# apache/arrow

Hardware: AMD Instinct MI355X
Metric: filter_take_mrows_per_s (higher is better)
Workload: dtype int64; 1 GPU; Filter+Take int64[1000000000] + validity (10% null), boolean mask 10% true, FilterOptions::DROP; take indices = the mask's row numbers (monotonic; indices_nonzero: uint64 through CallFunction, GetTakeIndices: uint32 in the mirror), no boundscheck; inputs = splitmix64 streams of SURVEY.md 8(d) (seeds 1,2,3); rows=1000000000, selected_rows=99992053, parallelism=single-gpu

## Files before the change

### arrow_amd/_lib.py

```python
from __future__ import annotations

import ctypes as C
import os

_HERE = os.path.dirname(os.path.abspath(__file__))
LIB_PATH = os.path.join(_HERE, "libarrow_amd.so")

ARX_OK = 0
ARX_OUT_OF_MEMORY = -1
ARX_INVALID = -4
ARX_CAPACITY_ERROR = -6
ARX_INDEX_ERROR = -7
ARX_NOT_IMPLEMENTED = -10
ARX_DEVICE_ERROR = -100

ABI_VERSION = 5

FILTER_DROP, FILTER_EMIT_NULL = 0, 1
JOIN_COLUMN, JOIN_LITERAL, JOIN_NULL = 0, 1, 2
JOIN_NULL_HANDLING = {"emit_null": 0, "skip": 1, "replace": 2}
JOIN_MAX_OPERANDS = 32
CASE_WHEN_MAX_CONDS = 16
ELEMENT_WISE_MIN, ELEMENT_WISE_MAX = 0, 1
ELEMENT_WISE_MAX_OPERANDS = 32
# ... 84 lines not shown
        ("kind", C.c_int32),
        ("reserved", C.c_int32),
        ("column", ArxBinarySpan),
        ("literal", C.c_void_p),
        ("literal_length", C.c_int64),
    ]


_p, _i64, _int, _u64, _u32, _sz = C.c_void_p, C.c_int64, C.c_int, C.c_uint64, C.c_uint32, C.c_size_t
_span = C.POINTER(ArxSpan)
_bspan = C.POINTER(ArxBinarySpan)

SIGNATURES = {
    "arx_last_error": (C.c_char_p, []),
    "arx_abi_version": (_int, []),
    "arx_device_count": (_int, []),
    "arx_set_option": (_int, [C.c_char_p, _i64]),
    "arx_get_option": (_int, [C.c_char_p, C.POINTER(_i64)]),
    "arx_get_counter": (_i64, [C.c_char_p]),
    "arx_filter_workspace_bytes": (_sz, [_i64]),
    "arx_filter_count": (_int, [_span, _int, _p, _sz, C.POINTER(_i64), _p]),
    "arx_filter_count_async": (_int, [_span, _int, _p, _sz, _p]),
    "arx_filter_count_nulls": (_int, [_span, _span, _int, _p, _sz, C.POINTER(_i64), C.POINTER(_i64), _p]),
    "arx_filter_exec": (_int, [_span, _int, _span, _int, _p, _i64, _p, _p, _p]),
    "arx_mask_to_indices": (_int, [_span, _int, _p, _i64, _int, _p, _p, _p]),
    "arx_filter_compact_form": (_int, [_int, _int, _int, _int, _i64, _i64]),
    "arx_take_workspace_bytes": (_sz, []),
    "arx_check_index_bounds": (_int, [_span, _int, _u64, _p, _sz, _p]),
    "arx_take": (_int, [_span, _int, _span, _int, _p, _p, _p, _p]),
    "arx_take_rows": (_int, [_span, _i64, _span, _int, _p, _p, _p, _p]),
    "arx_take_bits": (_int, [_span, _span, _int, _p, _p, _p, _p]),
    "arx_binary_take_workspace_bytes": (_sz, [_i64]),
    "arx_binary_take_offsets": (_int, [_bspan, _span, _int, _p, _sz, _p, _p, _p, C.POINTER(_i64), _p]),
    "arx_binary_take_data": (_int, [_bspan, _i64, _p, _sz, _p, _i64, _p, _p]),
    "arx_large_binary_take_workspace_bytes": (_sz, [_i64]),
    "arx_large_binary_take_offsets": (_int, [_bspan, _span, _int, _p, _sz, _p, _p, _p, C.POINTER(_i64), _p]),
    "arx_large_binary_take_data": (_int, [_bspan, _i64, _p, _sz, _p, _i64, _p, _p]),
    "arx_list_take_data": (_int, [_bspan, _int, _i64, _p, _sz, _p, _i64, _p, _p]),
    "arx_large_list_take_data": (_int, [_bspan, _int, _i64, _p, _sz, _p, _i64, _p, _p]),
    "arx_plain_byte_array_offsets": (_int, [_p, _sz, _i64, C.c_int32, _p]),
    "arx_rle_scan_runs": (_int, [_p, _sz, _int, _i64, _u32, _u64, _p, _i64, C.POINTER(_i64), C.POINTER(_i64)]),
    "arx_rle_decode_u32": (_int, [_p, _sz, _p, _i64, _int, _i64, _p, _p]),
    "arx_rle_decode_equals_bitmap": (_int, [_p, _sz, _p, _i64, _int, _i64, _u32, _p, _p]),
    "arx_expand_by_mask": (_int, [_p, _int, _span, _p, _p, _p]),
    "arx_rle_levels_to_bitmap": (_int, [_p, _p, _i64, _p, _p, _p, _p]),
    "arx_rle_scan_runs_equals": (_int, [_p, _sz, _int, _i64, _u32, _u32, _u64, _p, _i64, C.POINTER(_i64), C.POINTER(_i64)]),
# ... 210 lines not shown
```

### arrow_amd/csrc/plugin/common.inc

```

std::atomic<int64_t> g_gpu_calls{0};
std::atomic<int64_t> g_stock_calls{0};
std::atomic<int64_t> g_min_rows{1 << 16};
std::atomic<int64_t> g_min_rows_streaming{INT64_MAX};
std::atomic<int64_t> g_filter_morsel_rows{[] {
  const char* env = std::getenv("ARROW_AMD_FILTER_MORSEL_ROWS");
  return env != nullptr ? static_cast<int64_t>(std::strtoll(env, nullptr, 10)) : int64_t(1) << 20;
}()};

std::atomic<bool> g_parquet_pinned_staging{true};
std::atomic<bool> g_parquet_device_levels{true};
std::atomic<int> g_parquet_read_threads{4};
std::atomic<int64_t> g_parquet_read_part_bytes{int64_t(1) << 23};
std::atomic<bool> g_parquet_device_snappy{[] {
  const char* env = std::getenv("ARROW_AMD_PARQUET_DEVICE_SNAPPY");
  return env == nullptr || std::strtoll(env, nullptr, 10) != 0;
}()};
std::atomic<int64_t> g_parquet_device_snappy_pages{0};
std::atomic<bool> g_parquet_device_gzip{true};
std::atomic<int64_t> g_parquet_device_gzip_pages{0};
std::atomic<int64_t> g_parquet_copied_pages{0};

std::atomic<int64_t> g_aggregate_flush_rows{[] {
  const char* env = std::getenv("ARROW_AMD_AGGREGATE_FLUSH_ROWS");
// ... 70 lines not shown
    case ARX_CAPACITY_ERROR: return Status::CapacityError(msg);
    case ARX_INDEX_ERROR: return Status::IndexError(msg);
    case ARX_NOT_IMPLEMENTED: return Status::NotImplemented(msg);
    case ARX_OUT_OF_MEMORY: return Status::OutOfMemory(msg);
    default: return Status::UnknownError(msg);
  }
}

#define HIP_RETURN_NOT_OK(call)                                                        \
  do {                                                                                 \
    hipError_t e__ = (call);                                                           \
    if (e__ != hipSuccess)                                                             \
      return Status::IOError("HIP: ", hipGetErrorString(e__), " in " #call);           \
  } while (0)

thread_local hipStream_t t_stream = nullptr;

class DeviceScratch {
 public:
  ~DeviceScratch() {
    for (auto& s : slots_) {
      if (s.ptr) (void)hipFree(s.ptr);
    }
  }
  hipStream_t PeekStream() const { return stream_; }
  Status Stream(hipStream_t* out) {
    if (!stream_) {
      HIP_RETURN_NOT_OK(hipStreamCreateWithFlags(&stream_, hipStreamNonBlocking));
      t_stream = stream_;
    }
    *out = stream_;
    return Status::OK();
  }
  Status Get(int slot, size_t bytes, void** out) {
    if (slots_.size() <= static_cast<size_t>(slot)) slots_.resize(slot + 1);
    Slot& s = slots_[slot];
    bytes = (bytes + 255) & ~size_t(255);
    if (s.size < bytes) {
      if (s.ptr) HIP_RETURN_NOT_OK(hipFree(s.ptr));
      s.ptr = nullptr;
      s.size = 0;
      const size_t want = std::max<size_t>(bytes + bytes / 4, 1 << 20);
      HIP_RETURN_NOT_OK(hipMalloc(&s.ptr, want));
      s.size = want;
    }
    *out = s.ptr;
    return Status::OK();
  }

 private:
  struct Slot { void* ptr = nullptr; size_t size = 0; };
  std::vector<Slot> slots_;
  hipStream_t stream_ = nullptr;
};
thread_local DeviceScratch t_scratch;

class PinnedStaging {
 public:
  ~PinnedStaging() {
    if (ptr_) (void)hipHostFree(ptr_);
  }
  Status Reserve(size_t bytes, uint8_t** out) {
    if (size_ < bytes) {
      if (ptr_) HIP_RETURN_NOT_OK(hipHostFree(ptr_));
      ptr_ = nullptr;
      size_ = 0;
      const size_t want = std::max<size_t>(bytes + bytes / 4, size_t(1) << 20);
      HIP_RETURN_NOT_OK(hipHostMalloc(&ptr_, want, hipHostMallocDefault));
      size_ = want;
    }
    *out = static_cast<uint8_t*>(ptr_);
    return Status::OK();
  }
  void Trim(size_t keep_at_most) {
    if (size_ > keep_at_most && ptr_ != nullptr) {
      (void)hipHostFree(ptr_);
      ptr_ = nullptr;
      size_ = 0;
// ... 106 lines not shown
```

### arrow_amd/csrc/plugin/selection.inc

```
StockKernel g_stock_filter;

arrow::Result<std::unique_ptr<cp::KernelState>> FilterInit(cp::KernelContext* ctx,
                                                           const cp::KernelInitArgs& args) {
  auto state = std::make_unique<ShimState<cp::FilterOptions>>();
  if (g_stock_filter.init) {
    ARROW_ASSIGN_OR_RAISE(state->stock, g_stock_filter.init(ctx, args));
  }
  if (args.options != nullptr) {
    state->options = *static_cast<const cp::FilterOptions*>(args.options);
  }
  return state;
}

Status BooleanTakeOnDevice(const ArxSpan& dv, const ArxSpan& di, int tid, hipStream_t st, ArrayData* out_arr) {
  const int64_t m = di.length;
  const int64_t bytes = ((m + 63) / 64) * 8;
  const bool allocate_validity = dv.null_count != 0 || di.null_count != 0;
  out_arr->length = m;
  out_arr->buffers.resize(2);
  out_arr->buffers[0] = nullptr;
  ARROW_ASSIGN_OR_RAISE(out_arr->buffers[1], AllocDevice(bytes));
  void* d_valid = nullptr;
  void* d_counter = nullptr;
  if (allocate_validity) {
    ARROW_ASSIGN_OR_RAISE(out_arr->buffers[0], AllocDevice(bytes));
    d_valid = reinterpret_cast<void*>(out_arr->buffers[0]->mutable_address());
    ARROW_RETURN_NOT_OK(t_scratch.Get(kCounter, 64, &d_counter));
    HIP_RETURN_NOT_OK(hipMemsetAsync(d_counter, 0, 8, st));
  }
  ARROW_RETURN_NOT_OK(FromArx(arx_take_bits(&dv, &di, tid, reinterpret_cast<void*>(out_arr->buffers[1]->mutable_address()),
                                            d_valid, static_cast<int64_t*>(d_counter), st)));
  int64_t valid_count = m;
  if (allocate_validity) HIP_RETURN_NOT_OK(hipMemcpyAsync(&valid_count, d_counter, 8, hipMemcpyDeviceToHost, st));
  HIP_RETURN_NOT_OK(hipStreamSynchronize(st));
  out_arr->null_count = m - valid_count;
  return Status::OK();
}

bool ReeFilterOnRocm(const ArraySpan& filter) {
  return filter.type->id() == Type::RUN_END_ENCODED && filter.child_data.size() == 2 &&
         OnRocm(filter.child_data[0]) && OnRocm(filter.child_data[1]);
}
Status ExpandReeFilterOnDevice(const ArraySpan& filter, hipStream_t st, ArxSpan* dm) {
  const ArraySpan& run_ends = filter.child_data[0];
  const ArraySpan& run_values = filter.child_data[1];
  const int rw = FixedByteWidth(*run_ends.type);
  if (run_values.type->id() != Type::BOOL || (rw != 2 && rw != 4 && rw != 8)) {
    return Status::NotImplemented("arrow_amd: filter of type ", filter.type->ToString());
  }
  ArxSpan ends{}, vals{};
  ARROW_RETURN_NOT_OK(DeviceSpan(run_ends, &ends));
  ARROW_RETURN_NOT_OK(DeviceSpan(run_values, &vals));
  const int64_t n = filter.length;
  const size_t bytes = static_cast<size_t>((n + 63) / 64) * 8 + 64;
  void *d_bits = nullptr, *d_valid = nullptr;
  ARROW_RETURN_NOT_OK(t_scratch.Get(kArg2, bytes, &d_bits));
  const bool may_have_nulls = vals.validity != nullptr && vals.null_count != 0;
  if (may_have_nulls) ARROW_RETURN_NOT_OK(t_scratch.Get(kArg2Validity, bytes, &d_valid));
// ... 56 lines not shown
      ARROW_RETURN_NOT_OK(ExpandReeFilterOnDevice(filter, st, &dm));
    } else {
      ARROW_RETURN_NOT_OK(DeviceSpan(filter, &dm));
    }
    const size_t ws_bytes = arx_filter_workspace_bytes(filter.length);
    void* ws = nullptr;
    ARROW_RETURN_NOT_OK(t_scratch.Get(kWs, ws_bytes, &ws));
    ArrayData* out_arr = out->array_data().get();
    const bool allocate_validity = dv.null_count != 0 || dm.null_count != 0;
    if (filter.length > 0 && filter.length <= g_filter_morsel_rows.load()) {
      const int64_t n = filter.length;
      ARROW_RETURN_NOT_OK(FromArx(arx_filter_count_async(&dm, null_sel, ws, ws_bytes, st)));
      out_arr->buffers.resize(2);
      ARROW_ASSIGN_OR_RAISE(out_arr->buffers[1], AllocDevice(n * w));
      out_arr->buffers[0] = nullptr;
      void* d_valid = nullptr;
      if (allocate_validity) {
        ARROW_ASSIGN_OR_RAISE(out_arr->buffers[0], AllocDevice(((n + 63) / 64) * 8));
        d_valid = reinterpret_cast<void*>(out_arr->buffers[0]->mutable_address());
      }
      ARROW_RETURN_NOT_OK(FromArx(arx_filter_exec(&dv, w, &dm, null_sel, ws, n,
                                                  reinterpret_cast<void*>(out_arr->buffers[1]->mutable_address()),
                                                  d_valid, st)));
      int64_t selected = 0, set_bits = 0;
      HIP_RETURN_NOT_OK(hipMemcpyAsync(&selected, ws, 8, hipMemcpyDeviceToHost, st));
      if (allocate_validity) {
        void* cws = nullptr;
        ARROW_RETURN_NOT_OK(t_scratch.Get(kCounter, 64, &cws));
        ARROW_RETURN_NOT_OK(FromArx(arx_bitmap_popcount(d_valid, 0, n, cws, 64, &set_bits, st)));
      } else {
        HIP_RETURN_NOT_OK(hipStreamSynchronize(st));
      }
      out_arr->length = selected;
      out_arr->null_count = allocate_validity ? selected - set_bits : 0;
      static_cast<RocmBuffer*>(out_arr->buffers[1].get())->Shrink(selected * w);
      if (allocate_validity) static_cast<RocmBuffer*>(out_arr->buffers[0].get())->Shrink(((selected + 63) / 64) * 8);
      CountGpu(kFnFilter);
      return Status::OK();
    }
    int64_t out_len = 0, out_nulls = 0;
    if (allocate_validity) {
      ARROW_RETURN_NOT_OK(FromArx(arx_filter_count_nulls(&dv, &dm, null_sel, ws, ws_bytes, &out_len, &out_nulls, st)));
    } else {
      ARROW_RETURN_NOT_OK(FromArx(arx_filter_count(&dm, null_sel, ws, ws_bytes, &out_len, st)));
    }
    out_arr->length = out_len;
    out_arr->buffers.resize(2);
    ARROW_ASSIGN_OR_RAISE(out_arr->buffers[1], AllocDevice(out_len * w));
    out_arr->buffers[0] = nullptr;
    void* d_valid = nullptr;
    if (allocate_validity) {
      ARROW_ASSIGN_OR_RAISE(out_arr->buffers[0], AllocDevice(((out_len + 63) / 64) * 8));
      d_valid = reinterpret_cast<void*>(out_arr->buffers[0]->mutable_address());
    }
    ARROW_RETURN_NOT_OK(FromArx(arx_filter_exec(&dv, w, &dm, null_sel, ws, out_len,
                                                reinterpret_cast<void*>(out_arr->buffers[1]->mutable_address()),
                                                d_valid, st)));
    out_arr->null_count = allocate_validity ? out_nulls : 0;
    HIP_RETURN_NOT_OK(hipStreamSynchronize(st));
    CountGpu(kFnFilter);
    return Status::OK();
  }
  if (w == 0 || filter.type->id() != Type::BOOL || values.length < g_min_rows.load() ||
      !IsHost(values) || !IsHost(filter)) {
    return RunStock(kFnFilter, g_stock_filter, state->stock.get(), ctx, batch, out);
  }
  hipStream_t st;
  ARROW_RETURN_NOT_OK(t_scratch.Stream(&st));
// ... 258 lines not shown
    }
    if (w == 0 || tid < 0) {
      return Status::NotImplemented("arrow_amd: take of ", values.type->ToString(), " by ",
                                    indices.type->ToString(), " on device-resident arrays");
    }
    hipStream_t st;
    ARROW_RETURN_NOT_OK(t_scratch.Stream(&st));
    ArxSpan dv{}, di{};
    ARROW_RETURN_NOT_OK(DeviceSpan(values, &dv));
    ARROW_RETURN_NOT_OK(DeviceSpan(indices, &di));
    if (state->options.boundscheck) ARROW_RETURN_NOT_OK(CheckBoundsOnDevice(di, tid, values.length, st));
    const int64_t m = indices.length;
    const bool allocate_validity = dv.null_count != 0 || di.null_count != 0;
    ArrayData* out_arr = out->array_data().get();
    out_arr->length = m;
    out_arr->buffers.resize(2);
    ARROW_ASSIGN_OR_RAISE(out_arr->buffers[1], AllocDevice(m * w));
    out_arr->buffers[0] = nullptr;
    void* d_valid = nullptr;
    void* d_counter = nullptr;
    if (allocate_validity) {
      ARROW_ASSIGN_OR_RAISE(out_arr->buffers[0], AllocDevice(((m + 63) / 64) * 8));
      d_valid = reinterpret_cast<void*>(out_arr->buffers[0]->mutable_address());
      ARROW_RETURN_NOT_OK(t_scratch.Get(kCounter, 64, &d_counter));
      HIP_RETURN_NOT_OK(hipMemsetAsync(d_counter, 0, 8, st));
    }
    ARROW_RETURN_NOT_OK(FromArx(arx_take(&dv, w, &di, tid,
                                         reinterpret_cast<void*>(out_arr->buffers[1]->mutable_address()), d_valid,
                                         static_cast<int64_t*>(d_counter), st)));
    int64_t valid_count = m;
    if (allocate_validity) {
      HIP_RETURN_NOT_OK(hipMemcpyAsync(&valid_count, d_counter, 8, hipMemcpyDeviceToHost, st));
    }
    HIP_RETURN_NOT_OK(hipStreamSynchronize(st));
    out_arr->null_count = m - valid_count;
    CountGpu(kFnTake);
    return Status::OK();
  }
  if (w == 0 || tid < 0 || indices.length < g_min_rows.load() || !IsHost(values) || !IsHost(indices)) {
    return RunStock(kFnTake, g_stock_take, state->stock.get(), ctx, batch, out);
  }
  hipStream_t st;
  ARROW_RETURN_NOT_OK(t_scratch.Stream(&st));
  ArxSpan dv{}, di{};
  ARROW_RETURN_NOT_OK(Upload(values, w, kValues, kValidity, st, &dv));
  ARROW_RETURN_NOT_OK(Upload(indices, kIdxWidth[tid], kArg2, kArg2Validity, st, &di));
  if (state->options.boundscheck) ARROW_RETURN_NOT_OK(CheckBoundsOnDevice(di, tid, values.length, st));
  const int64_t m = indices.length;
  const bool allocate_validity = values.MayHaveNulls() || indices.MayHaveNulls();
  ArrayData* out_arr = out->array_data().get();
  out_arr->length = m;
  out_arr->buffers.resize(2);
  ARROW_ASSIGN_OR_RAISE(out_arr->buffers[1], ctx->Allocate(m * w));
  void* d_out = nullptr;
  void* d_out_valid = nullptr;
  void* d_counter = nullptr;
  ARROW_RETURN_NOT_OK(t_scratch.Get(kOutData, static_cast<size_t>(m) * w + 16, &d_out));
  if (allocate_validity) {
// ... 24 lines not shown
```

### arrow_amd/csrc/plugin/vector_hash.inc

```
enum HashVectorKind { kHashUnique = 0, kHashValueCounts, kHashDictEncode };

struct DeviceHashState : public cp::KernelState {
  HashVectorKind kind = kHashUnique;
  std::unique_ptr<cp::KernelState> stock;
  bool used_stock = false, used_device = false;
  bool encode_nulls = false;
  std::shared_ptr<arrow::DataType> type;
  int width = 0;
  std::shared_ptr<Buffer> table_buf, counts_buf;
  void* table = nullptr;
  int64_t max_groups = 0, num_groups = 0, counts_cap = 0;
};

StockKernel g_stock_unique, g_stock_value_counts, g_stock_dict_encode;
cp::VectorKernel::FinalizeFunc g_stock_unique_finalize = nullptr, g_stock_value_counts_finalize = nullptr,
                               g_stock_dict_encode_finalize = nullptr;

template <HashVectorKind KIND>
const StockKernel& StockHashKernel() {
  return KIND == kHashUnique ? g_stock_unique : KIND == kHashValueCounts ? g_stock_value_counts : g_stock_dict_encode;
}

Status HashUniques(DeviceHashState* s, hipStream_t st, std::shared_ptr<Buffer>* values, std::shared_ptr<Buffer>* validity,
                   int64_t* null_count) {
// ... 293 lines not shown
  } else {
    const int num = NonZeroNumericTypeId(in.type->id());
    if (num < 0) return Status::NotImplemented("arrow_amd: indices_nonzero of device-resident ", in.type->ToString(), " arrays");
    static const int widths[10] = {1, 1, 2, 2, 4, 4, 8, 8, 4, 8};
    ARROW_ASSIGN_OR_RAISE(bits, AllocDevice(((n + 63) / 64) * 8 + 8));
    const uint64_t zero = 0;
    const uint8_t* base = static_cast<const uint8_t*>(dv.data) + dv.offset * widths[num];
    if (n > 0) {
      ARROW_RETURN_NOT_OK(FromArx(arx_compare_numeric(ARX_CMP_NOT_EQUAL, num, base, nullptr, nullptr, &zero, n,
                                                      reinterpret_cast<uint64_t*>(bits->mutable_address()), st)));
    }
    dm.data = reinterpret_cast<const void*>(bits->address());
    dm.offset = 0;
    if (dm.validity != nullptr && dv.offset != 0) {
      ARROW_ASSIGN_OR_RAISE(rebased, AllocDevice(((n + 63) / 64) * 8 + 8));
      ARROW_RETURN_NOT_OK(FromArx(arx_bitmap_copy(dv.validity, dv.offset, n, reinterpret_cast<void*>(rebased->mutable_address()), st)));
      dm.validity = reinterpret_cast<const void*>(rebased->address());
    }
  }
  const size_t ws_bytes = arx_filter_workspace_bytes(n);
  void* ws = nullptr;
  ARROW_RETURN_NOT_OK(t_scratch.Get(kWs, ws_bytes, &ws));
  int64_t cnt = 0;
  if (n > 0) ARROW_RETURN_NOT_OK(FromArx(arx_filter_count(&dm, ARX_FILTER_DROP, ws, ws_bytes, &cnt, st)));
  void* d_idx = nullptr;
  ARROW_RETURN_NOT_OK(t_scratch.Get(kArg2, static_cast<size_t>(cnt) * 4 + 64, &d_idx));
  ARROW_ASSIGN_OR_RAISE(auto out_values, AllocDevice(std::max<int64_t>(cnt, 1) * 8));
  bool direct = false;
  if (cnt > 0) {
    direct = arx_mask_to_indices(&dm, ARX_FILTER_DROP, ws, cnt, 8, reinterpret_cast<void*>(out_values->mutable_address()), nullptr, st) == ARX_OK;
  }
  if (cnt > 0 && !direct) {
    ARROW_RETURN_NOT_OK(FromArx(arx_mask_to_indices(&dm, ARX_FILTER_DROP, ws, cnt, 4, d_idx, nullptr, st)));
    ArxSpan di{nullptr, d_idx, 0, cnt, 0};
    void* flag = nullptr;
    ARROW_RETURN_NOT_OK(t_scratch.Get(kFlag, 64, &flag));
    ARROW_RETURN_NOT_OK(FromArx(arx_cast_numeric(&di, ARX_NUM_UINT32, ARX_NUM_UINT64, 1, 1, flag, 64,
                                                 reinterpret_cast<void*>(out_values->mutable_address()), st)));
  }
  HIP_RETURN_NOT_OK(hipStreamSynchronize(st));
  CountGpu(kFnFilter);
  out->value = ArrayData::Make(arrow::uint64(), cnt, {nullptr, std::move(out_values)}, 0);
  return Status::OK();
}

Status RegisterIndicesNonZero(cp::FunctionRegistry* reg) {
  ARROW_ASSIGN_OR_RAISE(auto fn, reg->GetFunction("indices_nonzero"));
  if (fn->kind() != cp::Function::VECTOR) return Status::Invalid("indices_nonzero is not a vector function");
  auto* vfn = static_cast<cp::VectorFunction*>(fn.get());
  for (const auto& ty : {arrow::boolean(), arrow::int8(), arrow::uint8(), arrow::int16(), arrow::uint16(), arrow::int32(),
                         arrow::uint32(), arrow::int64(), arrow::uint64(), arrow::float32(), arrow::float64()}) {
    ARROW_ASSIGN_OR_RAISE(const cp::Kernel* k0, vfn->DispatchExact({ty}));
    cp::VectorKernel copy = *static_cast<const cp::VectorKernel*>(k0);
    if (g_stock_nonzero.exec == nullptr) g_stock_nonzero.exec = copy.exec;
    if (g_stock_nonzero.exec != copy.exec) continue;
// ... 64 lines not shown
```

### arrow_amd/csrc/selection.hip

```cpp
#include "arx_common.h"

#include <string.h>

#include <algorithm>
#include <type_traits>

namespace arx {

struct FilterWsHeader {
  int64_t total;
  int64_t ntiles;
  int64_t ngroups;
  int64_t length;
  int64_t valid;
  int64_t pad[3];
};
static_assert(sizeof(FilterWsHeader) == 64, "header is one 64-byte line");

struct FilterWsView {
  FilterWsHeader* hdr;
  int64_t* group_excl;
  int64_t* group_total;
  uint32_t* tile_counts;
  int64_t* group_valid;
// ... 10 lines not shown
  uint8_t* p = static_cast<uint8_t*>(ws);
  v.hdr = reinterpret_cast<FilterWsHeader*>(p);
  v.group_excl = reinterpret_cast<int64_t*>(p + 64);
  v.group_total = v.group_excl + ng;
  v.tile_counts = reinterpret_cast<uint32_t*>(v.group_total + ng);
  v.group_valid = reinterpret_cast<int64_t*>(v.tile_counts + ng * kTilesPerGroup);
  return v;
}

__device__ __forceinline__ uint64_t emit_word(const Bits& mask, const Bits& mvalid, int64_t w,
                                              bool emit_null, bool invert,
                                              uint64_t* mask_valid_out) {
  uint64_t m = load_word(mask, w);
  const uint64_t mv = load_word(mvalid, w);
  *mask_valid_out = mv;
  if (emit_null || invert) {
    const uint64_t in_range = load_word(Bits{nullptr, 0, mask.length, 0}, w);
    if (invert) m = ~m & in_range;
    if (emit_null) return (m | ~mv) & in_range;
  }
  return m & mv;
}

template <bool VALID>
__global__ __launch_bounds__(kBlock) void count_kernel(Bits mask, Bits mvalid, Bits vvalid, int emit_null,
                                                       int invert, int64_t ntiles,
                                                       uint32_t* tile_counts,
                                                       int64_t* group_total, int64_t* group_valid) {
  __shared__ uint32_t wave_sums[kWavesPerBlock];
  __shared__ uint32_t wave_valid[kWavesPerBlock];
  const int lane = lane_id();
  const int wave = threadIdx.x >> 6;
  const int64_t group = blockIdx.x;
  const int64_t t0 = group * kTilesPerGroup + wave * 16;
  uint32_t mine = 0;
  uint32_t kv = 0;
#pragma unroll 4
  for (int i = 0; i < 16; ++i) {
    const int64_t t = t0 + i;
    uint32_t k = 0;
    if (t < ntiles) {
      uint64_t mv;
      const uint64_t e = emit_word(mask, mvalid, t * 64 + lane, emit_null != 0, invert != 0, &mv);
      k = __popcll(e);
      if constexpr (VALID) kv += __popcll(e & mv & load_word(vvalid, t * 64 + lane));
    }
    const uint32_t s = wave_reduce_sum_u32(k);
    if (lane == i) mine = s;
  }
  if (lane < 16) tile_counts[t0 + lane] = mine;
  const uint32_t wsum = wave_reduce_sum_u32(lane < 16 ? mine : 0u);
  if (lane == 0) wave_sums[wave] = wsum;
  if constexpr (VALID) {
    const uint32_t vsum = wave_reduce_sum_u32(kv);
    if (lane == 0) wave_valid[wave] = vsum;
  }
  __syncthreads();
  if (threadIdx.x == 0) {
    int64_t s = 0, v = 0;
    for (int i = 0; i < kWavesPerBlock; ++i) {
      s += wave_sums[i];
      if constexpr (VALID) v += wave_valid[i];
    }
    group_total[group] = s;
    if constexpr (VALID) group_valid[group] = v;
  }
}

__global__ __launch_bounds__(1024) void scan_kernel(const int64_t* group_total, int64_t ngroups,
                                                    int64_t* group_excl, FilterWsHeader* hdr,
                                                    const int64_t* group_valid = nullptr) {
  __shared__ int64_t wave_tot[16];
  __shared__ int64_t carry_s;
  __shared__ unsigned long long valid_s;
  const int tid = threadIdx.x;
  const int lane = tid & 63;
  const int wave = tid >> 6;
  if (tid == 0) carry_s = 0;
  if (tid == 0) valid_s = 0;
  __syncthreads();
  if (group_valid != nullptr) {
    int64_t mine = 0;
    for (int64_t i = tid; i < ngroups; i += 1024) mine += group_valid[i];
#pragma unroll
    for (int d = 32; d >= 1; d >>= 1) mine += __shfl_xor(mine, d, 64);
    if (lane == 0 && mine != 0) atomicAdd(&valid_s, static_cast<unsigned long long>(mine));
    __syncthreads();
  }
  for (int64_t base = 0; base < ngroups; base += 1024) {
    const int64_t i = base + tid;
    const int64_t v = i < ngroups ? group_total[i] : 0;
    int64_t x = v;
#pragma unroll
    for (int d = 1; d < 64; d <<= 1) {
      const int64_t n = __shfl_up(x, d, 64);
      if (lane >= d) x += n;
    }
    if (lane == 63) wave_tot[wave] = x;
    __syncthreads();
    int64_t wave_prefix = 0;
    for (int k = 0; k < wave; ++k) wave_prefix += wave_tot[k];
    const int64_t carry = carry_s;
    if (i < ngroups) group_excl[i] = carry + wave_prefix + x - v;
    __syncthreads();
    if (tid == 1023) carry_s = carry + wave_prefix + x;
    __syncthreads();
  }
  if (tid == 0) {
    hdr->total = carry_s;
    hdr->valid = static_cast<int64_t>(valid_s);
  }
}

struct CompactArgs {
  const uint8_t* values;
  Bits mask;
  Bits mvalid;
  Bits vvalid;
  int64_t length;
  int64_t ntiles;
  const uint32_t* tile_counts;
  const int64_t* group_excl;
  uint8_t* out_data;
  uint64_t* out_validity;
  int emit_null;
  int invert;
  int values_aligned16;
};

constexpr int kFlushBytes = 2048;

template <int RING>
struct __attribute__((aligned(16))) CompactLds {
// ... 377 lines not shown


constexpr int kSparseWindow = 1024;
constexpr int kSparseU = 2;

struct __attribute__((aligned(16))) SparseLds {
  uint16_t sel[kWavesPerBlock][kSparseWindow];
  uint64_t vs[kWavesPerBlock][64];
  uint64_t zw[kWavesPerBlock][64];
};

template <int W, bool EMIT, bool IOTA>
__global__ __launch_bounds__(kBlock) void compact_sparse_kernel(CompactArgs a) {
  using E = typename ElemT<W>::type;
  constexpr int U = kSparseU;
  __shared__ SparseLds lds;

  const int lane = lane_id();
  const int wave = __builtin_amdgcn_readfirstlane(threadIdx.x >> 6);
  const int64_t t = static_cast<int64_t>(blockIdx.x) * kWavesPerBlock + wave;
  if (t >= a.ntiles) return;

  const int64_t w = t * 64 + lane;
  uint64_t mv;
  const uint64_t Ew = emit_word(a.mask, a.mvalid, w, EMIT, a.invert != 0, &mv);
  const uint32_t k = __popcll(Ew);
  const uint32_t incl = wave_inclusive_scan_u32(k);
  const uint32_t p = incl - k;
  const int total = static_cast<int>(__shfl(incl, 63, 64));
  if (total == 0) return;

  const int64_t grp = t >> 6;
  const int tin = static_cast<int>(t & 63);
  const uint32_t cprev = lane < tin ? a.tile_counts[grp * kTilesPerGroup + lane] : 0u;
  const int64_t off = a.group_excl[grp] + wave_reduce_sum_u32(cprev);

  uint16_t* sel = lds.sel[wave];
  const bool want_validity = a.out_validity != nullptr;
  if (want_validity) lds.vs[wave][lane] = load_word(a.vvalid, w) & mv;
  if constexpr (EMIT) lds.zw[wave][lane] = Ew & ~mv;

  const E* __restrict__ values = IOTA ? nullptr : reinterpret_cast<const E*>(a.values) + t * kTileRows;
  E* __restrict__ out = reinterpret_cast<E*>(a.out_data);
  const int head = static_cast<int>(off & 63);
  const int nsteps = (head + total + 63) >> 6;
  const int64_t word0 = off >> 6;
  constexpr int kStepsPerWindow = kSparseWindow / 64;

  uint64_t m = Ew;
  uint32_t rk = p;
  for (int step0 = 0; step0 < nsteps; step0 += kStepsPerWindow) {
    const int win_lo = step0 * 64 - head;
    const int win_hi = win_lo + kSparseWindow;
    while (m != 0 && static_cast<int>(rk) < win_hi) {
      const int bpos = __ffsll(static_cast<unsigned long long>(m)) - 1;
      m &= m - 1;
      sel[static_cast<int>(rk) - win_lo] = static_cast<uint16_t>(lane * 64 + bpos);
      ++rk;
    }
    wave_lds_sync();
    const int step_end = (step0 + kStepsPerWindow) < nsteps ? (step0 + kStepsPerWindow) : nsteps;
    const int first_listed = win_lo < 0 ? 0 : win_lo;
// ... 438 lines not shown
  return ARX_OK;
}

static inline const void* effective_validity(const ArxSpan* s) {
  return (s->null_count != 0) ? s->validity : nullptr;
}

static int launch_count(const ArxSpan* mask, int null_selection, void* ws, size_t ws_bytes,
                        hipStream_t st, int invert = 0, const ArxSpan* values = nullptr) {
  const int rc = check_mask(mask, null_selection);
  if (rc != ARX_OK) return rc;
  const size_t need = arx_filter_workspace_bytes(mask->length);
  if (ws == nullptr || ws_bytes < need) {
    set_error("filter workspace too small: %zu < %zu", ws_bytes, need);
    return ARX_INVALID;
  }
  if ((reinterpret_cast<uint64_t>(ws) & 63) != 0) {
    set_error("filter workspace must be 64-byte aligned");
    return ARX_INVALID;
  }
  FilterWsView v = ws_view(ws, mask->length);
  const int64_t nt = num_tiles(mask->length);
  const int64_t ng = num_groups(mask->length);
  FilterWsHeader h{};
  h.total = 0;
  h.ntiles = nt;
  h.ngroups = ng;
  h.length = mask->length;
  ARX_HIP(hipMemcpyAsync(v.hdr, &h, sizeof(h), hipMemcpyHostToDevice, st));
  if (mask->length == 0) return ARX_OK;
  const Bits mb = make_bits(mask->data, mask->offset, mask->length);
  const Bits mvb = make_bits(effective_validity(mask), mask->offset, mask->length);
  if (values != nullptr) {
    const Bits vvb = make_bits(effective_validity(values), values->offset, mask->length);
    hipLaunchKernelGGL((count_kernel<true>), dim3(static_cast<unsigned>(ng)), dim3(kBlock), 0, st, mb, mvb, vvb,
                       null_selection, invert, nt, v.tile_counts, v.group_total, v.group_valid);
    ARX_CHECK_LAUNCH("count_kernel");
    hipLaunchKernelGGL(scan_kernel, dim3(1), dim3(1024), 0, st, v.group_total, ng, v.group_excl, v.hdr,
                       static_cast<const int64_t*>(v.group_valid));
  } else {
    hipLaunchKernelGGL((count_kernel<false>), dim3(static_cast<unsigned>(ng)), dim3(kBlock), 0, st, mb, mvb, mvb,
                       null_selection, invert, nt, v.tile_counts, v.group_total, static_cast<int64_t*>(nullptr));
    ARX_CHECK_LAUNCH("count_kernel");
    hipLaunchKernelGGL(scan_kernel, dim3(1), dim3(1024), 0, st, v.group_total, ng, v.group_excl, v.hdr,
                       static_cast<const int64_t*>(nullptr));
  }
  ARX_CHECK_LAUNCH("scan_kernel");
  return ARX_OK;
}

static Knob<int> g_filter_batch{4};
static Knob<int> g_filter_pipe{1};
static Knob<int> g_filter_sparse{-1};
static const KnobRow kSelectionKnobs[] = {
    {"filter_batch", g_filter_batch, knob_snap_down<1, 4>},
    {"filter_pipe", g_filter_pipe, knob_bool},
    {"filter_sparse", g_filter_sparse, knob_tri},
};
KnobTable selection_knobs() { return knob_table(kSelectionKnobs); }

template <int W, bool IOTA, bool EMIT, bool ALIGNED>
static void launch_compact_e(const CompactArgs& a, unsigned grid, hipStream_t st) {
  constexpr int kIters = kTileRows / (kWave * (16 / W));
  constexpr int kBig = kIters >= 8 ? 4 : 2;
  if (ALIGNED && g_filter_batch >= 4 && g_filter_pipe) {
    hipLaunchKernelGGL((compact_kernel<W, IOTA, EMIT, ALIGNED, kBig, true>), dim3(grid),
                       dim3(kBlock), 0, st, a);
  } else {
    hipLaunchKernelGGL((compact_kernel<W, IOTA, EMIT, ALIGNED, 1, false>), dim3(grid), dim3(kBlock),
// ... 140 lines not shown
  a.emit_null = 0;
  a.invert = invert ? 1 : 0;
  a.values_aligned16 = 1;
  return launch_compact(true, 4, a, st);
}

}

using namespace arx;

extern "C" {

size_t arx_filter_workspace_bytes(int64_t length) {
  if (length < 0) length = 0;
  const int64_t ng = num_groups(length);
  return static_cast<size_t>(64 + ng * 16 + ng * kTilesPerGroup * 4 + ng * 8 + 64);
}

int arx_filter_count_async(const ArxSpan* mask, int null_selection, void* ws, size_t ws_bytes,
                           void* stream) {
  return launch_count(mask, null_selection, ws, ws_bytes, as_stream(stream));
}

int arx_filter_count_nulls(const ArxSpan* values, const ArxSpan* mask, int null_selection, void* ws, size_t ws_bytes,
                           int64_t* out_length, int64_t* out_null_count, void* stream) {
  if (out_length == nullptr || out_null_count == nullptr || values == nullptr) {
    set_error("values / out_length / out_null_count is NULL");
    return ARX_INVALID;
  }
  if (mask != nullptr && values->length != mask->length) {
    set_error("filter values and mask differ in length (%lld vs %lld)", static_cast<long long>(values->length),
              static_cast<long long>(mask->length));
    return ARX_INVALID;
  }
  hipStream_t st = as_stream(stream);
  const int rc = launch_count(mask, null_selection, ws, ws_bytes, st, 0, values);
  if (rc != ARX_OK) return rc;
  int64_t hdr[5] = {0, 0, 0, 0, 0};
  ARX_HIP(hipMemcpyAsync(hdr, ws, sizeof(hdr), hipMemcpyDeviceToHost, st));
  ARX_HIP(hipStreamSynchronize(st));
  *out_length = hdr[0];
  *out_null_count = mask->length == 0 ? 0 : hdr[0] - hdr[4];
  return ARX_OK;
}

int arx_filter_count(const ArxSpan* mask, int null_selection, void* ws, size_t ws_bytes,
                     int64_t* out_length, void* stream) {
  if (out_length == nullptr) {
    set_error("out_length is NULL");
    return ARX_INVALID;
  }
  hipStream_t st = as_stream(stream);
  const int rc = launch_count(mask, null_selection, ws, ws_bytes, st);
  if (rc != ARX_OK) return rc;
  int64_t total = 0;
  ARX_HIP(hipMemcpyAsync(&total, ws, sizeof(int64_t), hipMemcpyDeviceToHost, st));
  ARX_HIP(hipStreamSynchronize(st));
  *out_length = total;
  return ARX_OK;
// ... 489 lines not shown
```

### include/arrow_amd.h

```cpp
#ifndef ARROW_AMD_H_
#define ARROW_AMD_H_

#include <stddef.h>
#include <stdint.h>

#ifdef __cplusplus
extern "C" {
#endif

#define ARX_ABI_VERSION 5

typedef enum ArxStatus {
  ARX_OK = 0,
  ARX_OUT_OF_MEMORY = -1,
  ARX_INVALID = -4,
  ARX_CAPACITY_ERROR = -6,
  ARX_INDEX_ERROR = -7,
  ARX_NOT_IMPLEMENTED = -10,
  ARX_DEVICE_ERROR = -100
} ArxStatus;

enum { ARX_FILTER_DROP = 0, ARX_FILTER_EMIT_NULL = 1 };
enum { ARX_SORT_ASCENDING = 0, ARX_SORT_DESCENDING = 1 };
enum { ARX_NULLS_AT_START = 0, ARX_NULLS_AT_END = 1 };
// ... 9 lines not shown
  int64_t offset;
  int64_t length;
  int64_t null_count;
} ArxSpan;

const char* arx_last_error(void);
int arx_abi_version(void);
int arx_device_count(void);
int arx_set_option(const char* name, int64_t value);
int arx_get_option(const char* name, int64_t* out_value);
int64_t arx_get_counter(const char* name);


size_t arx_filter_workspace_bytes(int64_t length);

int arx_filter_count(const ArxSpan* mask, int null_selection, void* ws, size_t ws_bytes,
                     int64_t* out_length, void* stream);

int arx_filter_count_nulls(const ArxSpan* values, const ArxSpan* mask, int null_selection, void* ws, size_t ws_bytes,
                           int64_t* out_length, int64_t* out_null_count, void* stream);

int arx_filter_count_async(const ArxSpan* mask, int null_selection, void* ws,
                           size_t ws_bytes, void* stream);

int arx_filter_exec(const ArxSpan* values, int byte_width, const ArxSpan* mask,
                    int null_selection, const void* ws, int64_t out_length, void* out_data,
                    void* out_validity, void* stream);

int arx_mask_to_indices(const ArxSpan* mask, int null_selection, const void* ws,
                        int64_t out_length, int index_width, void* out_indices,
                        void* out_validity, void* stream);

enum { ARX_COMPACT_GATHER = 0, ARX_COMPACT_SWEEP_PIPELINED = 1, ARX_COMPACT_SWEEP_PLAIN = 2, ARX_COMPACT_SWEEP_UNALIGNED = 3 };

int arx_filter_compact_form(int row_numbers, int byte_width, int values_aligned16, int invert,
                            int64_t length, int64_t out_length);

size_t arx_take_workspace_bytes(void);

int arx_check_index_bounds(const ArxSpan* indices, int index_type, uint64_t upper_limit,
                           void* ws, size_t ws_bytes, void* stream);

int arx_take(const ArxSpan* values, int byte_width, const ArxSpan* indices, int index_type,
             void* out_data, void* out_validity, int64_t* valid_count, void* stream);

int arx_take_rows(const ArxSpan* values, int64_t row_bytes, const ArxSpan* indices, int index_type, void* out_data,
// ... 653 lines not shown
```

Baseline: 306,400 Mrows/s.

## Batch count-kernel loads, fold header init into scan, pin readbacks, elide counter memsets

Several changes land together. Device-to-host readbacks now go through a pinned host buffer instead of pageable stack variables. The host-to-device header copy is replaced by having the scan kernel write the whole header. The count kernel now issues its mask and validity word loads in batches of four tiles, and the scan kernel processes four groups per thread and folds the valid-count reduction into the same pass. The exec kernel also issues its tile-count and group-offset loads earlier, and a reusable device counter is re-zeroed after use so the next call can skip a memset. These aim to cut host-device synchronisation and transfer overhead and to raise memory-level parallelism in the count pass, at the cost of more code and more registers per thread.

```diff
diff --git a/arrow_amd/_lib.py b/arrow_amd/_lib.py
--- a/arrow_amd/_lib.py
+++ b/arrow_amd/_lib.py
@@ -130,6 +130,7 @@
     "arx_filter_count": (_int, [_span, _int, _p, _sz, C.POINTER(_i64), _p]),
     "arx_filter_count_async": (_int, [_span, _int, _p, _sz, _p]),
     "arx_filter_count_nulls": (_int, [_span, _span, _int, _p, _sz, C.POINTER(_i64), C.POINTER(_i64), _p]),
+    "arx_filter_count_nulls_async": (_int, [_span, _span, _int, _p, _sz, _p]),
     "arx_filter_exec": (_int, [_span, _int, _span, _int, _p, _i64, _p, _p, _p]),
     "arx_mask_to_indices": (_int, [_span, _int, _p, _i64, _int, _p, _p, _p]),
     "arx_filter_compact_form": (_int, [_int, _int, _int, _int, _i64, _i64]),
diff --git a/arrow_amd/csrc/plugin/common.inc b/arrow_amd/csrc/plugin/common.inc
--- a/arrow_amd/csrc/plugin/common.inc
+++ b/arrow_amd/csrc/plugin/common.inc
@@ -116,6 +116,8 @@
     for (auto& s : slots_) {
       if (s.ptr) (void)hipFree(s.ptr);
     }
+    if (readback_) (void)hipHostFree(readback_);
+    if (counter_) (void)hipFree(counter_);
   }
   hipStream_t PeekStream() const { return stream_; }
   Status Stream(hipStream_t* out) {
@@ -141,13 +143,45 @@
     *out = s.ptr;
     return Status::OK();
   }
+  Status Readback(int64_t** out) {
+    if (!readback_) HIP_RETURN_NOT_OK(hipHostMalloc(reinterpret_cast<void**>(&readback_), 64, hipHostMallocDefault));
+    *out = readback_;
+    return Status::OK();
+  }
+  Status ZeroCounter(hipStream_t st, void** out) {
+    if (!counter_) {
+      HIP_RETURN_NOT_OK(hipMalloc(&counter_, 256));
+      counter_is_zero_ = false;
+    }
+    if (!counter_is_zero_) HIP_RETURN_NOT_OK(hipMemsetAsync(counter_, 0, 8, st));
+    counter_is_zero_ = false;
+    *out = counter_;
+    return Status::OK();
+  }
+  Status CounterDone(hipStream_t st) {
+    HIP_RETURN_NOT_OK(hipMemsetAsync(counter_, 0, 8, st));
+    counter_is_zero_ = true;
+    return Status::OK();
+  }
 
  private:
   struct Slot { void* ptr = nullptr; size_t size = 0; };
   std::vector<Slot> slots_;
   hipStream_t stream_ = nullptr;
+  int64_t* readback_ = nullptr;
+  void* counter_ = nullptr;
+  bool counter_is_zero_ = false;
 };
 thread_local DeviceScratch t_scratch;
+
+Status ReadCountHeader(const void* ws, hipStream_t st, const int64_t** out) {
+  int64_t* host = nullptr;
+  ARROW_RETURN_NOT_OK(t_scratch.Readback(&host));
+  HIP_RETURN_NOT_OK(hipMemcpyAsync(host, ws, 5 * sizeof(int64_t), hipMemcpyDeviceToHost, st));
+  HIP_RETURN_NOT_OK(hipStreamSynchronize(st));
+  *out = host;
+  return Status::OK();
+}
 
 class PinnedStaging {
  public:
diff --git a/arrow_amd/csrc/plugin/selection.inc b/arrow_amd/csrc/plugin/selection.inc
--- a/arrow_amd/csrc/plugin/selection.inc
+++ b/arrow_amd/csrc/plugin/selection.inc
@@ -25,15 +25,18 @@
   if (allocate_validity) {
     ARROW_ASSIGN_OR_RAISE(out_arr->buffers[0], AllocDevice(bytes));
     d_valid = reinterpret_cast<void*>(out_arr->buffers[0]->mutable_address());
-    ARROW_RETURN_NOT_OK(t_scratch.Get(kCounter, 64, &d_counter));
-    HIP_RETURN_NOT_OK(hipMemsetAsync(d_counter, 0, 8, st));
+    ARROW_RETURN_NOT_OK(t_scratch.ZeroCounter(st, &d_counter));
   }
   ARROW_RETURN_NOT_OK(FromArx(arx_take_bits(&dv, &di, tid, reinterpret_cast<void*>(out_arr->buffers[1]->mutable_address()),
                                             d_valid, static_cast<int64_t*>(d_counter), st)));
-  int64_t valid_count = m;
-  if (allocate_validity) HIP_RETURN_NOT_OK(hipMemcpyAsync(&valid_count, d_counter, 8, hipMemcpyDeviceToHost, st));
+  int64_t* valid_count = nullptr;
+  ARROW_RETURN_NOT_OK(t_scratch.Readback(&valid_count));
+  if (allocate_validity) {
+    HIP_RETURN_NOT_OK(hipMemcpyAsync(valid_count, d_counter, 8, hipMemcpyDeviceToHost, st));
+    ARROW_RETURN_NOT_OK(t_scratch.CounterDone(st));
+  }
   HIP_RETURN_NOT_OK(hipStreamSynchronize(st));
-  out_arr->null_count = m - valid_count;
+  out_arr->null_count = allocate_validity ? m - valid_count[0] : 0;
   return Status::OK();
 }
 
@@ -136,8 +139,10 @@
       ARROW_RETURN_NOT_OK(FromArx(arx_filter_exec(&dv, w, &dm, null_sel, ws, n,
                                                   reinterpret_cast<void*>(out_arr->buffers[1]->mutable_address()),
                                                   d_valid, st)));
-      int64_t selected = 0, set_bits = 0;
-      HIP_RETURN_NOT_OK(hipMemcpyAsync(&selected, ws, 8, hipMemcpyDeviceToHost, st));
+      int64_t set_bits = 0;
+      int64_t* readback = nullptr;
+      ARROW_RETURN_NOT_OK(t_scratch.Readback(&readback));
+      HIP_RETURN_NOT_OK(hipMemcpyAsync(readback, ws, 8, hipMemcpyDeviceToHost, st));
       if (allocate_validity) {
         void* cws = nullptr;
         ARROW_RETURN_NOT_OK(t_scratch.Get(kCounter, 64, &cws));
@@ -145,6 +150,7 @@
       } else {
         HIP_RETURN_NOT_OK(hipStreamSynchronize(st));
       }
+      const int64_t selected = readback[0];
       out_arr->length = selected;
       out_arr->null_count = allocate_validity ? selected - set_bits : 0;
       static_cast<RocmBuffer*>(out_arr->buffers[1].get())->Shrink(selected * w);
@@ -152,12 +158,15 @@
       CountGpu(kFnFilter);
       return Status::OK();
     }
-    int64_t out_len = 0, out_nulls = 0;
     if (allocate_validity) {
-      ARROW_RETURN_NOT_OK(FromArx(arx_filter_count_nulls(&dv, &dm, null_sel, ws, ws_bytes, &out_len, &out_nulls, st)));
+      ARROW_RETURN_NOT_OK(FromArx(arx_filter_count_nulls_async(&dv, &dm, null_sel, ws, ws_bytes, st)));
     } else {
-      ARROW_RETURN_NOT_OK(FromArx(arx_filter_count(&dm, null_sel, ws, ws_bytes, &out_len, st)));
-    }
+      ARROW_RETURN_NOT_OK(FromArx(arx_filter_count_async(&dm, null_sel, ws, ws_bytes, st)));
+    }
+    const int64_t* counted = nullptr;
+    ARROW_RETURN_NOT_OK(ReadCountHeader(ws, st, &counted));
+    const int64_t out_len = counted[0];
+    const int64_t out_nulls = counted[0] - counted[4];
     out_arr->length = out_len;
     out_arr->buffers.resize(2);
     ARROW_ASSIGN_OR_RAISE(out_arr->buffers[1], AllocDevice(out_len * w));
@@ -462,18 +471,19 @@
     if (allocate_validity) {
       ARROW_ASSIGN_OR_RAISE(out_arr->buffers[0], AllocDevice(((m + 63) / 64) * 8));
       d_valid = reinterpret_cast<void*>(out_arr->buffers[0]->mutable_address());
-      ARROW_RETURN_NOT_OK(t_scratch.Get(kCounter, 64, &d_counter));
-      HIP_RETURN_NOT_OK(hipMemsetAsync(d_counter, 0, 8, st));
+      ARROW_RETURN_NOT_OK(t_scratch.ZeroCounter(st, &d_counter));
     }
     ARROW_RETURN_NOT_OK(FromArx(arx_take(&dv, w, &di, tid,
                                          reinterpret_cast<void*>(out_arr->buffers[1]->mutable_address()), d_valid,
                                          static_cast<int64_t*>(d_counter), st)));
-    int64_t valid_count = m;
+    int64_t* valid_count = nullptr;
+    ARROW_RETURN_NOT_OK(t_scratch.Readback(&valid_count));
     if (allocate_validity) {
-      HIP_RETURN_NOT_OK(hipMemcpyAsync(&valid_count, d_counter, 8, hipMemcpyDeviceToHost, st));
+      HIP_RETURN_NOT_OK(hipMemcpyAsync(valid_count, d_counter, 8, hipMemcpyDeviceToHost, st));
+      ARROW_RETURN_NOT_OK(t_scratch.CounterDone(st));
     }
     HIP_RETURN_NOT_OK(hipStreamSynchronize(st));
-    out_arr->null_count = m - valid_count;
+    out_arr->null_count = allocate_validity ? m - valid_count[0] : 0;
     CountGpu(kFnTake);
     return Status::OK();
   }
diff --git a/arrow_amd/csrc/plugin/vector_hash.inc b/arrow_amd/csrc/plugin/vector_hash.inc
--- a/arrow_amd/csrc/plugin/vector_hash.inc
+++ b/arrow_amd/csrc/plugin/vector_hash.inc
@@ -339,15 +339,20 @@
   void* ws = nullptr;
   ARROW_RETURN_NOT_OK(t_scratch.Get(kWs, ws_bytes, &ws));
   int64_t cnt = 0;
-  if (n > 0) ARROW_RETURN_NOT_OK(FromArx(arx_filter_count(&dm, ARX_FILTER_DROP, ws, ws_bytes, &cnt, st)));
-  void* d_idx = nullptr;
-  ARROW_RETURN_NOT_OK(t_scratch.Get(kArg2, static_cast<size_t>(cnt) * 4 + 64, &d_idx));
+  if (n > 0) {
+    ARROW_RETURN_NOT_OK(FromArx(arx_filter_count_async(&dm, ARX_FILTER_DROP, ws, ws_bytes, st)));
+    const int64_t* counted = nullptr;
+    ARROW_RETURN_NOT_OK(ReadCountHeader(ws, st, &counted));
+    cnt = counted[0];
+  }
   ARROW_ASSIGN_OR_RAISE(auto out_values, AllocDevice(std::max<int64_t>(cnt, 1) * 8));
   bool direct = false;
   if (cnt > 0) {
     direct = arx_mask_to_indices(&dm, ARX_FILTER_DROP, ws, cnt, 8, reinterpret_cast<void*>(out_values->mutable_address()), nullptr, st) == ARX_OK;
   }
   if (cnt > 0 && !direct) {
+    void* d_idx = nullptr;
+    ARROW_RETURN_NOT_OK(t_scratch.Get(kArg2, static_cast<size_t>(cnt) * 4 + 64, &d_idx));
     ARROW_RETURN_NOT_OK(FromArx(arx_mask_to_indices(&dm, ARX_FILTER_DROP, ws, cnt, 4, d_idx, nullptr, st)));
     ArxSpan di{nullptr, d_idx, 0, cnt, 0};
     void* flag = nullptr;
diff --git a/arrow_amd/csrc/selection.hip b/arrow_amd/csrc/selection.hip
--- a/arrow_amd/csrc/selection.hip
+++ b/arrow_amd/csrc/selection.hip
@@ -56,34 +56,81 @@
   return m & mv;
 }
 
+constexpr int kCountBatch = 4;
+constexpr int kTilesPerWave = kTilesPerGroup / kWavesPerBlock;
+static_assert(kTilesPerWave % kCountBatch == 0, "a wave's tiles are whole batches");
+
+template <int N>
+__device__ __forceinline__ void fetch_words(const Bits& b, int64_t w0, uint64_t (&lo)[N], uint64_t (&hi)[N]) {
+#pragma unroll
+  for (int i = 0; i < N; ++i) lo[i] = hi[i] = 0;
+  if (b.base == nullptr) return;
+  const int64_t last = b.nphys - 1;
+#pragma unroll
+  for (int i = 0; i < N; ++i) {
+    const int64_t w = w0 + i * 64;
+    lo[i] = b.base[w < last ? w : last];
+  }
+  if (b.shift != 0) {
+#pragma unroll
+    for (int i = 0; i < N; ++i) {
+      const int64_t w = w0 + i * 64 + 1;
+      hi[i] = b.base[w < last ? w : last];
+    }
+  }
+}
+
+__device__ __forceinline__ uint64_t fetched_word(const Bits& b, int64_t w, uint64_t lo, uint64_t hi) {
+  const int64_t remain = b.length - (w << 6);
+  const uint64_t in_range = remain >= 64 ? ~uint64_t(0) : (remain <= 0 ? uint64_t(0) : ((uint64_t(1) << remain) - 1));
+  const uint64_t v = b.base == nullptr ? ~uint64_t(0) : ((lo >> b.shift) | ((hi << 1) << (63 - b.shift)));
+  return v & in_range;
+}
+
+__device__ __forceinline__ uint64_t emit_fetched(const Bits& mask, const Bits& mvalid, int64_t w, uint64_t m_lo,
+                                                 uint64_t m_hi, uint64_t mv_lo, uint64_t mv_hi, bool emit_null,
+                                                 bool invert, uint64_t* mask_valid_out) {
+  uint64_t m = fetched_word(mask, w, m_lo, m_hi);
+  const uint64_t mv = fetched_word(mvalid, w, mv_lo, mv_hi);
+  *mask_valid_out = mv;
+  const uint64_t in_range = fetched_word(Bits{nullptr, 0, mask.length, 0}, w, 0, 0);
+  if (invert) m = ~m & in_range;
+  return emit_null ? ((m | ~mv) & in_range) : (m & mv);
+}
+
 template <bool VALID>
 __global__ __launch_bounds__(kBlock) void count_kernel(Bits mask, Bits mvalid, Bits vvalid, int emit_null,
-                                                       int invert, int64_t ntiles,
-                                                       uint32_t* tile_counts,
+                                                       int invert, uint32_t* tile_counts,
                                                        int64_t* group_total, int64_t* group_valid) {
   __shared__ uint32_t wave_sums[kWavesPerBlock];
   __shared__ uint32_t wave_valid[kWavesPerBlock];
   const int lane = lane_id();
   const int wave = threadIdx.x >> 6;
   const int64_t group = blockIdx.x;
-  const int64_t t0 = group * kTilesPerGroup + wave * 16;
+  const int64_t t0 = group * kTilesPerGroup + wave * kTilesPerWave;
+  const bool emit = emit_null != 0, inv = invert != 0;
   uint32_t mine = 0;
   uint32_t kv = 0;
-#pragma unroll 4
-  for (int i = 0; i < 16; ++i) {
-    const int64_t t = t0 + i;
-    uint32_t k = 0;
-    if (t < ntiles) {
+#pragma unroll 1
+  for (int b0 = 0; b0 < kTilesPerWave; b0 += kCountBatch) {
+    const int64_t w0 = (t0 + b0) * 64 + lane;
+    uint64_t m_lo[kCountBatch], m_hi[kCountBatch], mv_lo[kCountBatch], mv_hi[kCountBatch];
+    uint64_t vv_lo[kCountBatch], vv_hi[kCountBatch];
+    fetch_words(mask, w0, m_lo, m_hi);
+    fetch_words(mvalid, w0, mv_lo, mv_hi);
+    if constexpr (VALID) fetch_words(vvalid, w0, vv_lo, vv_hi);
+#pragma unroll
+    for (int i = 0; i < kCountBatch; ++i) {
+      const int64_t w = w0 + i * 64;
       uint64_t mv;
-      const uint64_t e = emit_word(mask, mvalid, t * 64 + lane, emit_null != 0, invert != 0, &mv);
-      k = __popcll(e);
-      if constexpr (VALID) kv += __popcll(e & mv & load_word(vvalid, t * 64 + lane));
-    }
-    const uint32_t s = wave_reduce_sum_u32(k);
-    if (lane == i) mine = s;
-  }
-  if (lane < 16) tile_counts[t0 + lane] = mine;
-  const uint32_t wsum = wave_reduce_sum_u32(lane < 16 ? mine : 0u);
+      const uint64_t e = emit_fetched(mask, mvalid, w, m_lo[i], m_hi[i], mv_lo[i], mv_hi[i], emit, inv, &mv);
+      if constexpr (VALID) kv += __popcll(e & mv & fetched_word(vvalid, w, vv_lo[i], vv_hi[i]));
+      const uint32_t s = wave_reduce_sum_u32(__popcll(e));
+      if (lane == b0 + i) mine = s;
+    }
+  }
+  if (lane < kTilesPerWave) tile_counts[t0 + lane] = mine;
+  const uint32_t wsum = wave_reduce_sum_u32(lane < kTilesPerWave ? mine : 0u);
   if (lane == 0) wave_sums[wave] = wsum;
   if constexpr (VALID) {
     const uint32_t vsum = wave_reduce_sum_u32(kv);
@@ -101,30 +148,33 @@
   }
 }
 
-__global__ __launch_bounds__(1024) void scan_kernel(const int64_t* group_total, int64_t ngroups,
-                                                    int64_t* group_excl, FilterWsHeader* hdr,
-                                                    const int64_t* group_valid = nullptr) {
-  __shared__ int64_t wave_tot[16];
+constexpr int kScanBlock = 1024;
+constexpr int kScanPerThread = 4;
+
+__global__ __launch_bounds__(kScanBlock) void scan_kernel(const int64_t* group_total, int64_t ngroups, int64_t ntiles,
+                                                          int64_t length, int64_t* group_excl, FilterWsHeader* hdr,
+                                                          const int64_t* group_valid) {
+  __shared__ int64_t wave_tot[kScanBlock / 64];
+  __shared__ int64_t wave_vtot[kScanBlock / 64];
   __shared__ int64_t carry_s;
-  __shared__ unsigned long long valid_s;
   const int tid = threadIdx.x;
   const int lane = tid & 63;
   const int wave = tid >> 6;
   if (tid == 0) carry_s = 0;
-  if (tid == 0) valid_s = 0;
   __syncthreads();
-  if (group_valid != nullptr) {
-    int64_t mine = 0;
-    for (int64_t i = tid; i < ngroups; i += 1024) mine += group_valid[i];
-#pragma unroll
-    for (int d = 32; d >= 1; d >>= 1) mine += __shfl_xor(mine, d, 64);
-    if (lane == 0 && mine != 0) atomicAdd(&valid_s, static_cast<unsigned long long>(mine));
-    __syncthreads();
-  }
-  for (int64_t base = 0; base < ngroups; base += 1024) {
-    const int64_t i = base + tid;
-    const int64_t v = i < ngroups ? group_total[i] : 0;
-    int64_t x = v;
+  int64_t vmine = 0;
+  for (int64_t base = 0; base < ngroups; base += kScanBlock * kScanPerThread) {
+    const int64_t i0 = base + static_cast<int64_t>(tid) * kScanPerThread;
+    int64_t v[kScanPerThread];
+    int64_t sum = 0;
+#pragma unroll
+    for (int j = 0; j < kScanPerThread; ++j) {
+      v[j] = (i0 + j) < ngroups ? group_total[i0 + j] : 0;
+      if (group_valid != nullptr) vmine += (i0 + j) < ngroups ? group_valid[i0 + j] : 0;
+    }
+#pragma unroll
+    for (int j = 0; j < kScanPerThread; ++j) sum += v[j];
+    int64_t x = sum;
 #pragma unroll
     for (int d = 1; d < 64; d <<= 1) {
       const int64_t n = __shfl_up(x, d, 64);
@@ -135,14 +185,29 @@
     int64_t wave_prefix = 0;
     for (int k = 0; k < wave; ++k) wave_prefix += wave_tot[k];
     const int64_t carry = carry_s;
-    if (i < ngroups) group_excl[i] = carry + wave_prefix + x - v;
+    int64_t run = carry + wave_prefix + x - sum;
+#pragma unroll
+    for (int j = 0; j < kScanPerThread; ++j) {
+      if ((i0 + j) < ngroups) group_excl[i0 + j] = run;
+      run += v[j];
+    }
     __syncthreads();
-    if (tid == 1023) carry_s = carry + wave_prefix + x;
+    if (tid == kScanBlock - 1) carry_s = carry + wave_prefix + x;
     __syncthreads();
   }
+#pragma unroll
+  for (int d = 32; d >= 1; d >>= 1) vmine += __shfl_xor(vmine, d, 64);
+  if (lane == 0) wave_vtot[wave] = vmine;
+  __syncthreads();
   if (tid == 0) {
+    int64_t valid = 0;
+    for (int k = 0; k < kScanBlock / 64; ++k) valid += wave_vtot[k];
     hdr->total = carry_s;
-    hdr->valid = static_cast<int64_t>(valid_s);
+    hdr->ntiles = ntiles;
+    hdr->ngroups = ngroups;
+    hdr->length = length;
+    hdr->valid = valid;
+    hdr->pad[0] = hdr->pad[1] = hdr->pad[2] = 0;
   }
 }
 
@@ -566,22 +631,27 @@
   if (t >= a.ntiles) return;
 
   const int64_t w = t * 64 + lane;
+  const int64_t grp = t >> 6;
+  const int tin = static_cast<int>(t & 63);
+  const bool want_validity = a.out_validity != nullptr;
+  const uint32_t craw = a.tile_counts[grp * kTilesPerGroup + lane];
+  const int64_t gex = a.group_excl[grp];
+  uint64_t m_lo[1], m_hi[1], mv_lo[1], mv_hi[1], vv_lo[1] = {0}, vv_hi[1] = {0};
+  fetch_words(a.mask, w, m_lo, m_hi);
+  fetch_words(a.mvalid, w, mv_lo, mv_hi);
+  if (want_validity) fetch_words(a.vvalid, w, vv_lo, vv_hi);
   uint64_t mv;
-  const uint64_t Ew = emit_word(a.mask, a.mvalid, w, EMIT, a.invert != 0, &mv);
+  const uint64_t Ew = emit_fetched(a.mask, a.mvalid, w, m_lo[0], m_hi[0], mv_lo[0], mv_hi[0], EMIT, a.invert != 0, &mv);
+  if (want_validity) lds.vs[wave][lane] = fetched_word(a.vvalid, w, vv_lo[0], vv_hi[0]) & mv;
+  const int64_t off = gex + wave_reduce_sum_u32(lane < tin ? craw : 0u);
+
   const uint32_t k = __popcll(Ew);
   const uint32_t incl = wave_inclusive_scan_u32(k);
   const uint32_t p = incl - k;
   const int total = static_cast<int>(__shfl(incl, 63, 64));
   if (total == 0) return;
 
-  const int64_t grp = t >> 6;
-  const int tin = static_cast<int>(t & 63);
-  const uint32_t cprev = lane < tin ? a.tile_counts[grp * kTilesPerGroup + lane] : 0u;
-  const int64_t off = a.group_excl[grp] + wave_reduce_sum_u32(cprev);
-
   uint16_t* sel = lds.sel[wave];
-  const bool want_validity = a.out_validity != nullptr;
-  if (want_validity) lds.vs[wave][lane] = load_word(a.vvalid, w) & mv;
   if constexpr (EMIT) lds.zw[wave][lane] = Ew & ~mv;
 
   const E* __restrict__ values = IOTA ? nullptr : reinterpret_cast<const E*>(a.values) + t * kTileRows;
@@ -1066,29 +1136,24 @@
   FilterWsView v = ws_view(ws, mask->length);
   const int64_t nt = num_tiles(mask->length);
   const int64_t ng = num_groups(mask->length);
-  FilterWsHeader h{};
-  h.total = 0;
-  h.ntiles = nt;
-  h.ngroups = ng;
-  h.length = mask->length;
-  ARX_HIP(hipMemcpyAsync(v.hdr, &h, sizeof(h), hipMemcpyHostToDevice, st));
-  if (mask->length == 0) return ARX_OK;
+  if (mask->length == 0) {
+    ARX_HIP(hipMemsetAsync(v.hdr, 0, sizeof(FilterWsHeader), st));
+    return ARX_OK;
+  }
   const Bits mb = make_bits(mask->data, mask->offset, mask->length);
   const Bits mvb = make_bits(effective_validity(mask), mask->offset, mask->length);
   if (values != nullptr) {
     const Bits vvb = make_bits(effective_validity(values), values->offset, mask->length);
     hipLaunchKernelGGL((count_kernel<true>), dim3(static_cast<unsigned>(ng)), dim3(kBlock), 0, st, mb, mvb, vvb,
-                       null_selection, invert, nt, v.tile_counts, v.group_total, v.group_valid);
-    ARX_CHECK_LAUNCH("count_kernel");
-    hipLaunchKernelGGL(scan_kernel, dim3(1), dim3(1024), 0, st, v.group_total, ng, v.group_excl, v.hdr,
-                       static_cast<const int64_t*>(v.group_valid));
+                       null_selection, invert, v.tile_counts, v.group_total, v.group_valid);
   } else {
     hipLaunchKernelGGL((count_kernel<false>), dim3(static_cast<unsigned>(ng)), dim3(kBlock), 0, st, mb, mvb, mvb,
-                       null_selection, invert, nt, v.tile_counts, v.group_total, static_cast<int64_t*>(nullptr));
-    ARX_CHECK_LAUNCH("count_kernel");
-    hipLaunchKernelGGL(scan_kernel, dim3(1), dim3(1024), 0, st, v.group_total, ng, v.group_excl, v.hdr,
-                       static_cast<const int64_t*>(nullptr));
-  }
+                       null_selection, invert, v.tile_counts, v.group_total, static_cast<int64_t*>(nullptr));
+  }
+  ARX_CHECK_LAUNCH("count_kernel");
+  hipLaunchKernelGGL(scan_kernel, dim3(1), dim3(kScanBlock), 0, st, static_cast<const int64_t*>(v.group_total), ng, nt,
+                     mask->length, v.group_excl, v.hdr,
+                     static_cast<const int64_t*>(values != nullptr ? v.group_valid : nullptr));
   ARX_CHECK_LAUNCH("scan_kernel");
   return ARX_OK;
 }
@@ -1275,19 +1340,28 @@
   return launch_count(mask, null_selection, ws, ws_bytes, as_stream(stream));
 }
 
+int arx_filter_count_nulls_async(const ArxSpan* values, const ArxSpan* mask, int null_selection, void* ws,
+                                 size_t ws_bytes, void* stream) {
+  if (values == nullptr) {
+    set_error("values is NULL");
+    return ARX_INVALID;
+  }
+  if (mask != nullptr && values->length != mask->length) {
+    set_error("filter values and mask differ in length (%lld vs %lld)", static_cast<long long>(values->length),
+              static_cast<long long>(mask->length));
+    return ARX_INVALID;
+  }
+  return launch_count(mask, null_selection, ws, ws_bytes, as_stream(stream), 0, values);
+}
+
 int arx_filter_count_nulls(const ArxSpan* values, const ArxSpan* mask, int null_selection, void* ws, size_t ws_bytes,
                            int64_t* out_length, int64_t* out_null_count, void* stream) {
   if (out_length == nullptr || out_null_count == nullptr || values == nullptr) {
     set_error("values / out_length / out_null_count is NULL");
     return ARX_INVALID;
   }
-  if (mask != nullptr && values->length != mask->length) {
-    set_error("filter values and mask differ in length (%lld vs %lld)", static_cast<long long>(values->length),
-              static_cast<long long>(mask->length));
-    return ARX_INVALID;
-  }
   hipStream_t st = as_stream(stream);
-  const int rc = launch_count(mask, null_selection, ws, ws_bytes, st, 0, values);
+  const int rc = arx_filter_count_nulls_async(values, mask, null_selection, ws, ws_bytes, stream);
   if (rc != ARX_OK) return rc;
   int64_t hdr[5] = {0, 0, 0, 0, 0};
   ARX_HIP(hipMemcpyAsync(hdr, ws, sizeof(hdr), hipMemcpyDeviceToHost, st));
diff --git a/include/arrow_amd.h b/include/arrow_amd.h
--- a/include/arrow_amd.h
+++ b/include/arrow_amd.h
@@ -55,6 +55,9 @@
 
 int arx_filter_count_async(const ArxSpan* mask, int null_selection, void* ws,
                            size_t ws_bytes, void* stream);
+
+int arx_filter_count_nulls_async(const ArxSpan* values, const ArxSpan* mask, int null_selection, void* ws,
+                                 size_t ws_bytes, void* stream);
 
 int arx_filter_exec(const ArxSpan* values, int byte_width, const ArxSpan* mask,
                     int null_selection, const void* ws, int64_t out_length, void* out_data,
```

After: 312,600 Mrows/s (median of 6 runs). +2.0%, better.
